# masafumiendo/benchnav

Measured on AMD Instinct MI355X. Metric: MPPI solve-steps/sec (K=1024,T=50,256x256 map), higher is better.
Workload: dtype f32

## Files before the change

benchnav_amd/csrc/mppi_capi.cpp:

```cpp
#include "mppi_handle.h"

#include <algorithm>
#include <atomic>
#include <cmath>
#include <chrono>
#include <cstdarg>
#include <cstdio>
#include <cstdlib>
#include <cstring>
#include <cerrno>
#include <sys/stat.h>
#include <fcntl.h>
#include <sys/file.h>
#include <unistd.h>
#include <map>
#include <mutex>
#include <string>
#include <vector>

namespace bn {
namespace host {

static bool wave_kernel_is_faster(const bn::SolveParams &p, size_t resident_role_wgs, int n_cus)
{
// ... 58 lines not shown
    case BN_BUF_USTAR: return B * T * 2 * 4;
    case BN_BUF_XSTAR: return B * (T + 1) * 3 * 4;
    case BN_BUF_MEAN: return B * T * 2 * 4;
    case BN_BUF_MAP: return (size_t)h->n_maps * G * G * 4;
    case BN_BUF_GOAL: return B * 2 * 4;
    case BN_BUF_USTAR_XSTAR: return (B * T * 2 + B * (T + 1) * 3) * 4;
    default: return 0;
    }
}

int ensure_scratch(bn_mppi *h, size_t bytes)
{
    if (bytes <= h->scratch_bytes) return BN_OK;
    if (h->d_scratch) BN_HIP(hipFree(h->d_scratch));
    h->d_scratch = nullptr;
    h->scratch_bytes = 0;
    BN_HIP(hipMalloc(&h->d_scratch, bytes));
    h->scratch_bytes = bytes;
    return BN_OK;
}

int flush_tail(bn_mppi *h, float *out_copy)
{
    if (h->shard_tail_inflight) {
        BN_HIP(hipStreamWaitEvent(h->stream, h->ev_shard_tail[h->shard_tail_slot], 0));
        h->shard_tail_inflight = false;
    }
    if (!h->tail_pending) return BN_OK;
    bn::SolveParams p = h->p;
    p.out_copy = out_copy;
    const int cur3 = (int)((h->solves - 1) % kSlots);
    p.part = h->d_part[cur3]; p.cost = h->d_cost[cur3]; p.state = h->d_state_copy[cur3];
    if (h->ticket_mode) {
        p.tail_merged = 1;
        p.ustar_prev = h->d_ustar2[cur3]; p.stats_prev = h->d_stats2[cur3];
    }
    p.tail_solve = h->solves - 1;
    if (h->in_episode) {
        p.env_on = 1;
        p.ep_index = h->ep_len - 1;
        p.env_z = h->ep_z ? h->ep_z + (size_t)(h->ep_len - 1) * p.B : nullptr;
    }
    p.flag_tail = h->d_flags + kSlots * (size_t)p.B * bn::kFlagStride;
    h->tails += 1;
    if (h->overlap_used) p.err_dev = reinterpret_cast<int *>(h->d_flags + ((kSlots + 1) * (size_t)p.B + 2) * bn::kFlagStride);
    if (int rc = guard_foreign_overlap(h)) return rc;
    BN_HIP(bn::launch_finish(p, h->stream));
    h->tail_pending = false;
    return BN_OK;
}

int check_instance(const bn_mppi *h, int32_t instance, bool allow_all)
{
    if (!h) return fail(BN_ERR_INVALID, "null handle");
    if (instance == -1 && allow_all) return BN_OK;
    if (instance < 0 || instance >= h->p.B)
        return fail(BN_ERR_INVALID, "instance %d out of range [0,%d)", instance, h->p.B);
    return BN_OK;
}

void journal_arm_states(bn_mppi *h)
{
    if (h->replaying) return;
    h->snap_slot = h->journal.size();
    h->arm_state_snap = h->snap_slot < h->snap_cap;
}

void journal_push(bn_mppi *h, bn_mppi::BatchRec r, bool replayable)
{
    if (h->replaying) return;
    if (!h->last_batch_overlapped && h->journal.empty()) return;
    if (!replayable || h->journal.size() >= std::min(kJournalCap, h->snap_cap) || h->snap_slot != h->journal.size()) { h->journal_lost = true; h->journal.clear(); return; }
    r.states = h->d_state_snaps + h->snap_slot * (size_t)h->p.B * 3;
    if (!h->journal_lost) h->journal.push_back(r);
}

static int recover_overlap(bn_mppi *h)
{
    for (int q = 0; q < kMaxStreams - 1; ++q)
        if (h->xstream[q]) BN_HIP(hipStreamSynchronize(h->xstream[q]));
    BN_HIP(hipStreamSynchronize(h->stream));
    BN_HIP(hipMemset(h->d_flags, 0, ((kSlots + 1) * (size_t)h->p.B + 3) * bn::kFlagStride * sizeof(unsigned long long)));
    if (h->d_ticket) BN_HIP(hipMemset(h->d_ticket, 0, (size_t)h->p.B * 65 * 4));
    for (int q = 0; q < kSlots; ++q) h->pub[q] = 0;
    h->tails = 0;
    h->prev_published = false;
    h->tail_pending = false;
#ifdef BN_EXPERIMENTS
    fprintf(stderr, "[bn] expired wait: counter %d (B=%d: [slot][b] below %d, tails above) need %d seen %d | solve %d block (%d,%d) have_prev/overlap/cur_slot %d wait_part*1000+wait_tail %d | host: solves %llu tails %llu pub %llu %llu %llu %llu\n",
            h->h_err[8], h->p.B, kSlots * h->p.B, h->h_err[9], h->h_err[10], h->h_err[11], h->h_err[12], h->h_err[13], h->h_err[14], h->h_err[15],
            (unsigned long long)h->solves, (unsigned long long)h->tails, (unsigned long long)h->pub[0], (unsigned long long)h->pub[1], (unsigned long long)h->pub[2], (unsigned long long)h->pub[kSlots - 1]);
#endif
    h->overlap_off = true;
    h->overlap_used = false;
    h->arm_snap = false;
    h->arm_state_snap = false;
    h->in_episode = false;
    *h->h_err = 0;
    std::vector<bn_mppi::BatchRec> recs;
    recs.swap(h->journal);
    const bool lost = h->journal_lost || recs.empty();
    h->journal_lost = false;
    if (lost)
        return fail(BN_ERR_HIP, "an overlapped launch gave up waiting for its predecessor's partials and the batches since the last "
                                "synchronisation point cannot be re-run: their results are invalid; this handle runs its launches on one "
                                "stream from now on");
    BN_HIP(hipMemcpy(h->d_mean, h->d_mean_snap, (size_t)h->p.B * h->p.T * 2 * 4, hipMemcpyDeviceToDevice));
    h->solves = h->journal_solves0;
    h->replaying = true;
    int rc = BN_OK;
    for (const auto &r : recs) {
        rc = r.episode ? bn_mppi_episode_async(h, r.n, r.states, BN_MEM_DEVICE, r.eps, r.noise, r.eps_ring, r.eps_stride, r.z)
                       : bn_mppi_solve_n_async(h, r.n, r.states, BN_MEM_DEVICE, r.eps, r.noise, r.eps_ring, r.eps_stride);
        if (rc != BN_OK) break;
    }
    if (rc == BN_OK) rc = flush_tail(h);
    h->replaying = false;
    if (rc != BN_OK) return rc;
    BN_HIP(hipStreamSynchronize(h->stream));
    h->recoveries += 1;
    (void)fail(BN_OK, "warning: an overlapped launch gave up waiting for its predecessor's partials; %zu batch(es) were re-run on one "
                      "stream (results are valid now; this handle no longer overlaps its launches)", recs.size());
    return BN_OK;
}

static int settle_overlap(bn_mppi *h, bool synced)
{
    if (!h->overlap_used || h->replaying) return BN_OK;
    if (__atomic_load_n(h->h_err, __ATOMIC_ACQUIRE) == 0) {
        if (synced) {
            bool idle = true;
            for (int q = 0; idle && q + 1 < h->n_streams; ++q) idle = hipStreamQuery(h->xstream[q]) == hipSuccess;
            (void)hipGetLastError();
            if (idle) { h->overlap_used = false; h->journal.clear(); h->journal_lost = false; }
        }
        return BN_OK;
    }
    return recover_overlap(h);
}

static int sync_checked(bn_mppi *h)
{
    BN_HIP(hipStreamSynchronize(h->stream));
    if (h->overlap_used)
        for (int q = 0; q + 1 < h->n_streams; ++q)
            if (h->xstream[q]) BN_HIP(hipStreamSynchronize(h->xstream[q]));
    return settle_overlap(h, true);
}

int self_check(bn_mppi *h)
{
    if (!h->self_used || h->overlap_used || h->replaying) return BN_OK;
    if (__atomic_load_n(h->h_err, __ATOMIC_ACQUIRE) == 0) return BN_OK;
    BN_HIP(hipStreamSynchronize(h->stream));
    BN_HIP(hipMemset(h->d_flags, 0, ((kSlots + 1) * (size_t)h->p.B + 3) * bn::kFlagStride * sizeof(unsigned long long)));
    for (int q = 0; q < kSlots; ++q) h->pub[q] = 0;
    h->tails = 0;
    *h->h_err = 0;
    h->self_used = false;
    h->self_off = true;
    return fail(BN_ERR_HIP, "the tail of a one-launch solve gave up waiting for the rollout workgroups of its own launch: the outputs of solve %llu "
                            "are invalid (solve again); this handle goes back to two launches per synchronous solve",
                (unsigned long long)h->solves - 1);
}

int settle_point(bn_mppi *h)
// ... 209 lines not shown
    }
    alloc(&h->d_cost_out, B * K * 4);
    alloc(&h->d_w, B * K * 4);
    alloc(&h->d_ustar, (B * T * 2 + B * (T + 1) * 3) * 4);
    if (h->d_ustar) h->d_xstar = h->d_ustar + B * T * 2;
    alloc(&h->d_stats, B * 2 * 4);
    if (rc == BN_OK && hipHostMalloc((void **)&h->h_pinned, B * 3 * 4, hipHostMallocDefault) != hipSuccess)
        rc = fail(BN_ERR_HIP, "hipHostMalloc failed");
    if (rc == BN_OK) {
        if (!(cfg->flags & BN_FLAG_PRIVATE_STREAM)) {
            h->stream = (hipStream_t)cfg->stream;
        } else if (hipStreamCreateWithFlags(&h->stream, hipStreamNonBlocking) == hipSuccess) {
            h->own_stream = true;
        } else {
            rc = fail(BN_ERR_HIP, "hipStreamCreate failed");
        }
    }
    if (rc != BN_OK) {
        bn_mppi_destroy(h);
        return rc;
    }
    p.map = h->d_map; p.state = h->d_state; p.goal = h->d_goal; p.mean = h->d_mean; p.eps = nullptr;
    p.X = h->d_X; p.U = h->d_U; p.cost = h->d_cost[0]; p.part = h->d_part[0]; p.w = h->d_w;
    p.state_copy = h->d_state_copy[0]; p.cost_out = h->d_cost_out;
    p.ustar = h->d_ustar; p.xstar = h->d_xstar; p.stats = h->d_stats; p.mean_used = h->d_mean_used;
    p.slip_on = (cfg->flags & BN_FLAG_SAMPLED_SLIP) ? 1 : 0;
    if (p.slip_on && bn::sampled_fused(p)) h->resident_wgs = bn::sampled_resident_per_cu(p) * (size_t)h->n_cus;
    h->pipelined = !h->slow_path && !(cfg->flags & BN_FLAG_NO_PIPELINE) && p.nblk <= kPipelinedMaxBlocks && !p.slip_on;
    h->wave_kernel = h->pipelined && want_wave;
    h->lat_kernel = h->pipelined && !h->wave_kernel && !(cfg->flags & BN_FLAG_ROLE_KERNEL) && bn::lat_lds_bytes(p) > 0 &&
                    ((cfg->flags & BN_FLAG_LAT_KERNEL) || ((size_t)p.B + 1) * (p.nblk + 1) <= (size_t)std::max(prop.multiProcessorCount, 1));
    if (const char *e = exp_env("BN_LAT_KERNEL")) h->lat_kernel = h->lat_kernel && e[0] != '0';
    alloc(&h->d_flags, ((kSlots + 1) * B + 3) * bn::kFlagStride * sizeof(unsigned long long));
    alloc(&h->d_mean_snap, B * T * 2 * 4);
    if (rc == BN_OK) {
        if (hipHostMalloc((void **)&h->h_err, 64, hipHostMallocMapped) != hipSuccess) rc = fail(BN_ERR_HIP, "hipHostMalloc (error word) failed");
        else if (hipHostGetDevicePointer((void **)&h->d_err, h->h_err, 0) != hipSuccess) rc = fail(BN_ERR_HIP, "hipHostGetDevicePointer failed");
        else *h->h_err = 0;
    }
    if (rc == BN_OK) {
        if (hipHostMalloc((void **)&h->h_mail, B * 2 * sizeof(unsigned long long), hipHostMallocMapped) != hipSuccess ||
            hipHostGetDevicePointer((void **)&h->d_mail, h->h_mail, 0) != hipSuccess) rc = fail(BN_ERR_HIP, "hipHostMalloc (first-action mailbox) failed");
        else std::memset(h->h_mail, 0, B * 2 * sizeof(unsigned long long));
    }
    p.mail = h->d_mail;
    if (h->lat_kernel && p.nblk <= 16 && 2 * p.T <= bn::kRolloutThreads && !exp_env("BN_NO_GRANULES"))
        for (int q = 0; q < kSlots; ++q) alloc(&h->d_gran[q], (B * (size_t)p.nblk * (2 + 2 * T) + 4 * B) * sizeof(unsigned long long));
    h->role_overlap = h->pipelined && !h->lat_kernel && !(cfg->flags & BN_FLAG_NO_OVERLAP);
    if (const char *e = exp_env("BN_ROLE_OVERLAP")) h->role_overlap = h->role_overlap && e[0] != '0';
    const bool ticket_det = !h->slow_path && !p.slip_on && !h->pipelined && !(cfg->flags & BN_FLAG_NO_PIPELINE) && p.nblk <= 1024 &&
                            bn::finish_lds_bytes(p) + 256 <= bn::rollout_lds_bytes(p);
    h->ticket_overlap = (ticket_det || (!(cfg->flags & BN_FLAG_NO_PIPELINE) && bn::sampled_fused(p))) && !(cfg->flags & BN_FLAG_NO_OVERLAP) &&
                        !exp_env("BN_NO_TICKET_OVERLAP");
    const bool may_overlap = (h->lat_kernel || h->role_overlap || h->ticket_overlap) && !(cfg->flags & BN_FLAG_NO_OVERLAP);
    if (may_overlap) {
        h->n_streams = 2;
        if (const char *e = exp_env("BN_OVERLAP_STREAMS")) h->n_streams = std::min(std::max(std::atoi(e), 2), kMaxStreams);
        for (int q = 0; q + 1 < h->n_streams; ++q) {
            if (h->d_X) alloc(&h->d_Xalt[q], B * (T + 1) * 3 * (size_t)p.Kp * 4);
            if (h->d_U) alloc(&h->d_Ualt[q], B * T * 2 * (size_t)p.Kp * 4);
        }
        h->snap_cap = std::max<size_t>(64, std::min<size_t>(4096, ((size_t)16 << 20) / ((size_t)B * 12)));
        alloc(&h->d_state_snaps, h->snap_cap * B * 3 * 4);
    }
    if (rc == BN_OK && may_overlap) {
        bool ok = hipEventCreateWithFlags(&h->ev_fork, hipEventDisableTiming) == hipSuccess;
        for (int q = 0; ok && q < h->n_streams; ++q) ok = hipEventCreateWithFlags(&h->ev_guard[q], hipEventDisableTiming) == hipSuccess;
        for (int q = 0; ok && q + 1 < h->n_streams; ++q)
            ok = hipStreamCreateWithFlags(&h->xstream[q], hipStreamNonBlocking) == hipSuccess &&
                 hipEventCreateWithFlags(&h->ev_join[q], hipEventDisableTiming) == hipSuccess;
        if (!ok) rc = fail(BN_ERR_HIP, "stream / event creation for overlapped launches failed");
    }
    if (p.slip_on) {
        alloc(&h->d_slip_std, (size_t)h->n_maps * p.G * p.G * 4);
        p.slip_std = h->d_slip_std;
        for (int q = 0; q < kSlots; ++q) {
            alloc(&h->d_ustar2[q], (size_t)p.B * p.T * 2 * 4);
            alloc(&h->d_stats2[q], (size_t)p.B * 2 * 4);
        }
        alloc(&h->d_ticket, (size_t)p.B * 65 * 4);
        alloc(&h->d_gpart, (size_t)p.B * 64 * (2 + 2 * p.T) * 4);
        p.ticket = h->d_ticket; p.gpart = h->d_gpart;
        h->ticket_mode = !h->slow_path && !(cfg->flags & BN_FLAG_NO_PIPELINE) && bn::sampled_fused(p);
    } else if (ticket_det) {
        for (int q = 0; q < kSlots; ++q) {
            alloc(&h->d_ustar2[q], (size_t)p.B * p.T * 2 * 4);
            alloc(&h->d_stats2[q], (size_t)p.B * 2 * 4);
        }
        alloc(&h->d_ticket, (size_t)p.B * 65 * 4);
        alloc(&h->d_gpart, (size_t)p.B * 64 * (2 + 2 * p.T) * 4);
        p.gpart = h->d_gpart;
        h->ticket_mode = true;
    }
    if (rc == BN_OK && !p.pow2) {
        unsigned long long *bad = h->d_flags + ((kSlots + 1) * B + 1) * bn::kFlagStride;
        const float d_max = std::max(p.x_hi - p.x0, p.y_hi - p.y0);
        unsigned long long n_bad = 1;
        if (!(std::isfinite(d_max) && d_max >= 0.0f) || bn::launch_quotient_check(p.res, p.inv_res, d_max, bad, nullptr) != hipSuccess ||
            hipMemcpy(&n_bad, bad, sizeof n_bad, hipMemcpyDeviceToHost) != hipSuccess) {
            (void)hipGetLastError();
            rc = fail(BN_ERR_HIP, "checking the cell-index quotient for resolution %g failed", (double)p.res);
        } else if (n_bad != 0) {
            rc = fail(BN_ERR_INVALID, "resolution %.9g: the correctly rounded three-instruction quotient disagrees with the division for %llu "
                                      "positions in [0, %g] (no such resolution was known: please report it); use a neighbouring value",
                      (double)p.res, n_bad, (double)d_max);
        } else {
            p.fast_div = 1;
        }
        (void)hipMemset(bad, 0, sizeof n_bad);
    }
    if (rc == BN_OK && hipDeviceSynchronize() != hipSuccess) rc = fail(BN_ERR_HIP, "hipDeviceSynchronize failed after allocation");
    if (rc == BN_OK && may_overlap) {
        int *probe = reinterpret_cast<int *>(h->d_flags + ((kSlots + 1) * B + 1) * bn::kFlagStride);
        for (int q = 0; rc == BN_OK && q + 1 < h->n_streams; ++q) {
            bool found = false;
            for (int attempt = 0; attempt < 8; ++attempt) {
                int seen = 0;
                if (hipMemset(probe, 0, 2 * sizeof(int)) != hipSuccess || bn::launch_queue_probe(probe, h->stream, h->xstream[q], h->n_cus) != hipSuccess ||
                    hipStreamSynchronize(h->stream) != hipSuccess || hipStreamSynchronize(h->xstream[q]) != hipSuccess ||
                    hipMemcpy(&seen, probe + 1, sizeof seen, hipMemcpyDeviceToHost) != hipSuccess) {
                    (void)hipGetLastError();
                    rc = fail(BN_ERR_HIP, "probing the streams of overlapped launches failed");
                    break;
                }
                if (seen) { found = true; break; }
                if (attempt == 7) break;
                hipStream_t fresh = nullptr;
                if (hipStreamCreateWithFlags(&fresh, hipStreamNonBlocking) != hipSuccess) { (void)hipGetLastError(); break; }
                h->parked.push_back(h->xstream[q]);
                h->xstream[q] = fresh;
            }
            if (exp_env("BN_DEBUG_CREATE")) std::fprintf(stderr, "[bn_mppi_create] extra stream %d: %s after %zu replacement(s)\n", q, found ? "dispatches concurrently" : "NO concurrent queue found", h->parked.size());
            if (!found && rc == BN_OK) h->overlap_off = true;
        }
        (void)hipMemset(probe, 0, 2 * sizeof(int));
    }
    if (rc == BN_OK) rc = paced_setup(h, may_overlap);
    if (rc != BN_OK) {
        bn_mppi_destroy(h);
        return rc;
    }
    {
        std::lock_guard<std::mutex> lock(g_overlap_mu);
        g_handles[h->cfg.device_id].push_back(h);
    }
    *out = h;
    return BN_OK;
}

void bn_mppi_destroy(bn_mppi_t *h)
{
    if (!h) return;
    DeviceGuard guard(h->cfg.device_id);
    hp_cancel(h);
    (void)hipStreamSynchronize(h->stream);
    {
        std::lock_guard<std::mutex> lock(g_overlap_mu);
        auto it = g_overlap_owner.find(h->cfg.device_id);
        if (it != g_overlap_owner.end() && it->second == h) g_overlap_owner.erase(it);
        g_overlap_owners.store((int)g_overlap_owner.size(), std::memory_order_relaxed);
        auto &v = g_handles[h->cfg.device_id];
        v.erase(std::remove(v.begin(), v.end(), h), v.end());
    }
    for (hipEvent_t e : h->ev) (void)hipEventDestroy(e);
    if (h->shard_comm || h->shard_prepared) shard_comm_release(h);
    env_release(h);
// ... 264 lines not shown
            p.overlap = 0;
            h->pub[cur3] += (unsigned long long)p.nblk;
            p.self_tail = 1;
            p.wait_part_self = h->pub[cur3];
            p.wait_tail_self = h->tails;
            h->tails += 1;
            p.out_copy_self = h->self_out_copy;
            if (exp_env("BN_NO_EARLY_MAIL")) p.no_early_mail = 1;
            if (h->inline_state && p.B == 1) { p.state_inline = 1; p.sv0 = h->inline_state[0]; p.sv1 = h->inline_state[1]; p.sv2 = h->inline_state[2]; }
            h->self_used = true;
            h->self_tail_launched = true;
            h->prev_published = false;
            h->hp_gran_valid = p.gran != nullptr;
            h->x_idx = 0;
        } else
        if ((h->lat_kernel || h->role_overlap) && overlap) {
            p.flag_part = h->d_flags;
            p.err = h->d_err; p.err_dev = reinterpret_cast<int *>(h->d_flags + ((kSlots + 1) * B + 2) * bn::kFlagStride);
            if (h->arm_snap) { p.mean_snap = h->d_mean_snap; h->arm_snap = false; }
            p.cur_slot = cur3; p.prev_slot = prev3;
            p.wait_part = h->pub[prev3];
            p.gran = p.lat_kernel ? h->d_gran[cur3] : nullptr;
            if (alt_buffers) {
                if (h->d_Xalt[alt_buffers - 1]) p.X = h->d_Xalt[alt_buffers - 1];
                if (h->d_Ualt[alt_buffers - 1] && p.U) p.U = h->d_Ualt[alt_buffers - 1];
            }
            p.overlap = (h->prev_published && p.have_prev) ? 1 : 0;
            p.gran_prev = (p.overlap && p.lat_kernel) ? h->d_gran[prev3] : nullptr;
            if (on_stream) st = on_stream;
            if (p.overlap) h->overlap_used = true;
            h->pub[cur3] += (unsigned long long)p.nblk;
            h->prev_published = true;
            if (self_tail && p.lat_kernel && !h->in_episode) {
                p.self_tail = 1;
                p.wait_part_self = h->pub[cur3];
                p.wait_tail_self = h->tails;
                h->tails += 1;
            }
        } else {
            h->prev_published = false;
        }
        p.aux_prio = (!p.wave_kernel && (size_t)p.B * (p.nblk + 1) > h->resident_wgs) ? 1 : 0;
        if (!p.wave_kernel && !p.store_u) p.U = nullptr;
        if (p.self_tail) BN_HIP(bn::launch_rollout_lat_self(p, mode, st));
        else BN_HIP(bn::launch_rollout(p, mode, st));
        if (st != h->stream && lone_self) {
            BN_HIP(hipEventRecord(h->hp_ev[h->hp_redo_q], st));
            BN_HIP(hipStreamWaitEvent(h->stream, h->hp_ev[h->hp_redo_q], 0));
        }
        if (prof_grouped) h->prof_in_group = (h->prof_in_group + 1) % kProfGroup;
        h->solves += 1;
        h->x_idx = 0;
        h->tail_pending = !p.self_tail;
        if (p.self_tail) h->prev_published = false;
        if (lone_self) h->last_batch_overlapped = false;
        return BN_OK;
    }
    if (!(h->ticket_overlap && overlap && !shard_rollout)) h->prev_published = false;
    p.have_prev = 0;
    p.mean_from_part = 0;
    p.tail_solve = p.solve;
    if (p.slip_on && !h->slip_std_set) return fail(BN_ERR_STATE, "bn_mppi_set_slip_std must precede solve in sampled-slip mode");
    if (h->ticket_mode && !shard_rollout) {
        p.have_prev = h->tail_pending ? 1 : 0;
        p.tail_merged = 1;
        p.tail_solve = p.solve - 1;
        p.ustar_cur = h->d_ustar2[cur3]; p.stats_cur = h->d_stats2[cur3];
        p.ustar_prev = h->d_ustar2[prev3]; p.stats_prev = h->d_stats2[prev3];
        p.ticket = h->d_ticket;
        hipStream_t st = h->stream;
        p.flag_tail = h->d_flags + kSlots * B * bn::kFlagStride;
        if (p.have_prev) { p.wait_tail = h->tails; h->tails += 1; }
        if (h->ticket_overlap && overlap) {
            p.flag_part = h->d_flags;
            p.err = h->d_err; p.err_dev = reinterpret_cast<int *>(h->d_flags + ((kSlots + 1) * B + 2) * bn::kFlagStride);
            if (h->arm_snap) { p.mean_snap = h->d_mean_snap; h->arm_snap = false; }
            p.cur_slot = cur3; p.prev_slot = prev3;
            p.wait_part = h->pub[prev3];
            if (alt_buffers) {
                if (h->d_Xalt[alt_buffers - 1]) p.X = h->d_Xalt[alt_buffers - 1];
                if (h->d_Ualt[alt_buffers - 1] && p.U) p.U = h->d_Ualt[alt_buffers - 1];
            }
            p.overlap = (h->prev_published && p.have_prev) ? 1 : 0;
            if (on_stream) st = on_stream;
            if (p.overlap) h->overlap_used = true;
            h->pub[cur3] += 1;
            h->prev_published = true;
        }
        if (p.slip_on) BN_HIP(bn::launch_rollout_sampled(p, mode, st));
        else BN_HIP(bn::launch_rollout(p, mode, st));
        if (prof_grouped) h->prof_in_group = (h->prof_in_group + 1) % kProfGroup;
        h->solves += 1;
        h->tail_pending = true;
        return BN_OK;
    }
    if (shard_rollout && h->shard_inplace) p.part = h->d_gathered + (size_t)h->shard_rank * p.nblk * (2 + 2 * T);
    if (p.slip_on) {
        BN_HIP(bn::launch_rollout_sampled(p, mode, h->stream));
    } else {
        if (h->slow_path) p.wave_kernel = 1;
        else if (!p.store_u) p.U = nullptr;
        BN_HIP(bn::launch_rollout(p, mode, h->stream));
    }
    if (prof) BN_HIP(hipEventRecord(ev[1], h->stream));
    if (shard_rollout) {
        if (prof) BN_HIP(hipEventRecord(ev[2], h->stream));
        h->solves += 1;
        h->tail_pending = false;
        h->shard_pending = true;
        return BN_OK;
    }
    p.state = p.state_copy;
    BN_HIP(bn::launch_finish(p, h->stream));
    if (prof) BN_HIP(hipEventRecord(ev[2], h->stream));
    h->solves += 1;
    h->tail_pending = false;
    return BN_OK;
}

}
}

extern "C" {

int bn_mppi_solve_async(bn_mppi_t *h, const float *states, bn_mem_kind states_where, const float *eps,
                        bn_noise_kind noise)
{
    if (h && !h->replaying && !h->journal.empty()) {
        h->last_batch_overlapped = false;
        journal_arm_states(h);
        journal_push(h, bn_mppi::BatchRec{1, states, eps, noise, 1, 0, false, nullptr}, states_where == BN_MEM_DEVICE && noise != BN_NOISE_HOST_KT2);
    }
    return solve_impl(h, states, states_where, eps, noise, false);
}

int bn_mppi_solve_n_async(bn_mppi_t *h, int32_t n, const float *states, bn_mem_kind states_where, const float *eps,
                          bn_noise_kind noise, int32_t eps_ring, int64_t eps_stride)
{
    if (n < 0) return fail(BN_ERR_INVALID, "n must be >= 0");
    if (eps && (eps_ring < 1 || eps_stride < 0)) return fail(BN_ERR_INVALID, "eps_ring must be >= 1 and eps_stride >= 0");
    if (!h) return fail(BN_ERR_INVALID, "null handle");
    const bool overlap = (h->lat_kernel || h->role_overlap || h->ticket_overlap) && h->n_streams > 1 && (h->d_Xalt[0] || h->p.lean) && n >= 3 && states_where == BN_MEM_DEVICE &&
                         noise != BN_NOISE_HOST_KT2 && !(h->cfg.flags & (BN_FLAG_PROFILE | BN_FLAG_NO_OVERLAP)) && !h->shard_pending && !h->overlap_off;
    int mode = overlap ? h->tune.chosen : 1;
    if (overlap && h->tune.explore && n >= 128 && !h->in_episode && !h->replaying) {
        const int32_t ring = eps ? eps_ring : 1;
        const int32_t prefix = ((192 + ring - 1) / ring) * ring;
        if (n > prefix + 2) {
            if (int rc = bn_mppi_solve_n_async(h, prefix, states, states_where, eps, noise, eps_ring, eps_stride)) return rc;
            h->tune.explore = 0;
            return bn_mppi_solve_n_async(h, n - prefix, states, states_where, eps, noise, eps_ring, eps_stride);
        }
        mode = 1 - h->tune.chosen;
    }
    if (mode != h->run_mode) h->ov_sample.valid = false;
    h->run_mode = mode;
    bool mine = overlap && mode == 0;
    if (mine) {
        BN_BIND(h);
        std::lock_guard<std::mutex> lock(g_overlap_mu);
        bn_mppi *&owner = g_overlap_owner[h->cfg.device_id];
        if (owner && owner != h) {
            bool busy = hipStreamQuery(owner->stream) != hipSuccess;
            for (int q = 0; !busy && q + 1 < owner->n_streams; ++q) busy = hipStreamQuery(owner->xstream[q]) != hipSuccess;
            (void)hipGetLastError();
            if (busy) mine = false;
// ... 162 lines not shown
```

benchnav_amd/csrc/rollout_sampled.hip:

```cpp
#include "mppi_device.h"

namespace bn {

namespace {

constexpr int kSampledWaves = 8;
constexpr int kSampledThreads = 64 * kSampledWaves;

__host__ __device__ inline size_t sampled_lds_floats(int T, int WN)
{
    const size_t TP = (size_t)((T + 2) & ~1);
    return 4 * 64 * (size_t)(T + 1) + 2 * (size_t)WN * WN + 2 * 64 * TP + 2 * (size_t)T * kUPad + 4 * (size_t)T + 128;
}

template <int EPS, int GEO, bool STORE_U>
__global__ __launch_bounds__(kSampledThreads) void rollout_sampled_kernel(const SolveParams p)
{
    extern __shared__ __attribute__((aligned(16))) float smem[];
    const int T = p.T, K = p.K, WN2 = p.WN * p.WN;
    const int TP = (T + 2) & ~1;
    float4 *XL = reinterpret_cast<float4 *>(smem);
    float2 *win2 = reinterpret_cast<float2 *>(smem + 4 * 64 * (T + 1));
    float *Zt = reinterpret_cast<float *>(win2 + WN2), *Zc = Zt + 64 * TP;
    float *Ul = Zc + 64 * TP, *ml = Ul + 2 * T * kUPad, *mv = ml + 2 * T, *el = mv + 2 * T, *ad = el + 64;
    const WgId wg = decode_wg(p);
    if (wg.idle) return;
    const int tid = threadIdx.x, lane = tid & 63, b = wg.b;
    if (wg.aux) {
        if (p.overlap) finish_body<GEO, true, kSampledThreads, false, true>(p, b, nullptr, p.cost_prev, p.state_prev, smem);
        else finish_body<GEO, true, kSampledThreads>(p, b, nullptr, p.cost_prev, p.state_prev, smem);
        return;
    }
    const int wid = __builtin_amdgcn_readfirstlane(tid >> 6);
    const int k = wg.blk * 64 + lane;
    const bool active = k < K;
    const int kk = active ? k : K - 1;
    const float *__restrict__ mu = p.map + (size_t)b * p.map_stride;
    const float *__restrict__ sg = p.slip_std + (size_t)b * p.map_stride;
    const float sx = p.state[b * 3 + 0], sy = p.state[b * 3 + 1], sth = p.state[b * 3 + 2];
    const float gx = p.goal[b * 2 + 0], gy = p.goal[b * 2 + 1];
    const Win w = window_origin<GEO>(p, sx, sy);
    const size_t Kp = (size_t)p.Kp;
    float *Xb = p.X + (size_t)b * (T + 1) * 3 * Kp + k;
    float *Ub = STORE_U ? p.U + (size_t)b * T * 2 * Kp + k : nullptr;

    BN_STAMP(0);
    for (int e = tid; e < WN2; e += kSampledThreads) {
        const int r = e / p.WN, c = e - r * p.WN;
        const size_t g = (size_t)min(w.wy0 + r, p.G - 1) * p.G + min(w.wx0 + c, p.G - 1);
        win2[e] = make_float2(mu[g], sg[g]);
    }
    const bool ovs = p.overlap != 0;
    const bool tpub = p.flag_part != nullptr;
    if (!ovs)
    for (int j = tid; j < 2 * T; j += kSampledThreads) {
        const float m = p.mean[(size_t)b * 2 * T + j];
        ml[j] = m;
        mv[j] = m * ((j & 1) ? p.iv1 : p.iv0);
    }
    if (wg.blk == 0 && tid < 3) { if (tpub) store_agent(p.state_copy + b * 3 + tid, p.state[b * 3 + tid]); else p.state_copy[b * 3 + tid] = p.state[b * 3 + tid]; }
    if (p.state_snap && wg.blk == 0 && tid < 3) p.state_snap[b * 3 + tid] = p.state[b * 3 + tid];
    __syncthreads();

    {
        const int nE = (T + 1) >> 1, nS = TP >> 1;
        for (int q = nE + wid; q < nE + nS; q += kSampledWaves) {
            {
                const int r0 = 2 * (q - nE), r1 = r0 + 1;
                float z[4];
                if (p.zt) {
                    z[0] = r0 < T ? p.zt[((size_t)b * T + r0) * K + kk] : 0.0f;
                    z[1] = r1 < T ? p.zt[((size_t)b * T + r1) * K + kk] : 0.0f;
                    z[2] = r0 <= T ? p.zc[((size_t)b * (T + 1) + r0) * K + kk] : 0.0f;
                    z[3] = r1 <= T ? p.zc[((size_t)b * (T + 1) + r1) * K + kk] : 0.0f;
                } else {
                    philox_slip_block(p.seed, p.solve, (uint32_t)b, (uint32_t)(kk + p.k0), (uint32_t)(q - nE), z);
                }
                Zt[r0 * 64 + lane] = z[0]; Zt[r1 * 64 + lane] = z[1];
                Zc[r0 * 64 + lane] = z[2]; Zc[r1 * 64 + lane] = z[3];
            }
        }
        if (ovs) {
            if (tid == 0) wait_counter<16>(flag_ctr(p.flag_part, p.prev_slot * p.B + b), p.wait_part, p);
            __syncthreads();
            for (int j = tid; j < 2 * T; j += kSampledThreads) {
                const float m = load_agent(p.mean + (size_t)b * 2 * T + j);
                ml[j] = m;
                mv[j] = m * ((j & 1) ? p.iv1 : p.iv0);
            }
            __syncthreads();
        }
        if (p.mean_snap && wg.blk == 0 && wid == 0) snapshot_mean(p, b, ml, lane);
        for (int q = wid; q < nE; q += kSampledWaves) produce_pair<EPS, STORE_U>(p, p.eps, b, kk, 2 * q, p.solve, ml, Ul, Ub, Kp, lane);
    }
    __syncthreads();
    BN_STAMP(1);

    if (wid == 0) {
        SlipChain c;
        c.x = sx; c.y = sy; c.th = sth;
        sincos_spec(c.th, c.sn, c.cs);
        c.e = slip_cell_safe<GEO, true>(p, w, sx, sy);
        float xn, yn, tn;
        slip_chain_step<GEO, true>(p, win2, w, c, Ul[lane], Ul[kUPad + lane], Zt[lane], xn, yn, tn);
        XL[lane] = make_float4(xn, yn, tn, __int_as_float(c.e));
        int t = 1;
        for (; t + 4 <= T; t += 4) {
            float uq[4][3];
#pragma unroll
            for (int i = 0; i < 4; ++i) {
                uq[i][0] = Ul[(2 * (t + i)) * kUPad + lane]; uq[i][1] = Ul[(2 * (t + i) + 1) * kUPad + lane];
                uq[i][2] = Zt[(t + i) * 64 + lane];
            }
#pragma unroll
            for (int i = 0; i < 4; ++i) {
                slip_chain_step<GEO, false>(p, win2, w, c, uq[i][0], uq[i][1], uq[i][2], xn, yn, tn);
                __builtin_amdgcn_sched_barrier(0);
                XL[(t + i) * 64 + lane] = make_float4(xn, yn, tn, __int_as_float(c.e));
            }
        }
        for (; t < T; ++t) {
            slip_chain_step<GEO, false>(p, win2, w, c, Ul[(2 * t) * kUPad + lane], Ul[(2 * t + 1) * kUPad + lane], Zt[t * 64 + lane],
                                        xn, yn, tn);
            XL[t * 64 + lane] = make_float4(xn, yn, tn, __int_as_float(c.e));
        }
        XL[T * 64 + lane] = make_float4(c.x, c.y, c.th, __int_as_float(c.e));
    } else if (wid == 1) {
        double Ad = 0.0;
        for (int t = 0; t < T; ++t)
            Ad += (double)(p.lambda_ * (mv[2 * t] * Ul[(2 * t) * kUPad + lane] + mv[2 * t + 1] * Ul[(2 * t + 1) * kUPad + lane]));
        ad[lane] = (float)Ad;
    }
    __syncthreads();
    BN_STAMP(2);

    for (int t = wid; t <= T; t += kSampledWaves) {
        const float4 o = XL[t * 64 + lane];
        float *Xt = Xb + (size_t)(3 * t) * Kp;
        Xt[0] = o.x; Xt[Kp] = o.y; Xt[2 * Kp] = o.z;
        const float2 ms = win2[__float_as_int(o.w)];
        const float tc = trav_from_slip(ms.x, ms.y, Zc[t * 64 + lane]);
        const float dx = o.x - gx, dy = o.y - gy;
        Zc[t * 64 + lane] = sqrt_cr_normal(dx * dx + dy * dy) + (tc <= p.thr ? 1.0e4f : 0.0f);
    }
    __syncthreads();
    BN_STAMP(3);

    if (wid == 0) {
        double Sd = 0.0;
#pragma unroll 16
        for (int t = 0; t < T; ++t) Sd += (double)Zc[t * 64 + lane];
        const float cost = ((float)Sd + Zc[T * 64 + lane]) + ad[lane];
        if (active) { if (tpub) store_agent(p.cost + (size_t)b * K + k, cost); else p.cost[(size_t)b * K + k] = cost; }
        const float zz = active ? (-cost) / p.lambda_ : -INFINITY;
        const float zmax = wave_max(zz);
        const float e = active ? expf(zz - zmax) : 0.0f;
        const float esum = wave_sum(e);
        el[lane] = e;
        if (lane == 0) {
            float *part = p.part + ((size_t)b * p.nblk + wg.blk) * (2 + 2 * T);
            store_agent(part, zmax); store_agent(part + 1, esum);
        }
    }
    __syncthreads();
    column_sums<kSampledThreads, true>(Ul, el, T, tid, p.part + ((size_t)b * p.nblk + wg.blk) * (2 + 2 * T));
    BN_STAMP(5);
    if (p.ustar_cur) ticket_merge<kSampledThreads>(p, b, wg.blk, smem);
}

template <int EPS, int GEO, bool STORE_U>
__global__ __launch_bounds__(64) void rollout_sampled_global_kernel(const SolveParams p)
{
    extern __shared__ __attribute__((aligned(16))) float smem[];
    const int T = p.T, K = p.K;
    float *ml = smem, *mv = ml + 2 * T, *Ul = mv + 2 * T, *el = Ul + 2 * T * kUPad;
    const WgId wg = decode_wg(p);
    if (wg.idle) return;
    const int lane = threadIdx.x, b = wg.b;
    const int k = wg.blk * 64 + lane;
    const bool active = k < K;
    const int kk = active ? k : K - 1;
    const float *__restrict__ mu = p.map + (size_t)b * p.map_stride;
    const float *__restrict__ sg = p.slip_std + (size_t)b * p.map_stride;
    const float sx = p.state[b * 3 + 0], sy = p.state[b * 3 + 1], sth = p.state[b * 3 + 2];
    const float gx = p.goal[b * 2 + 0], gy = p.goal[b * 2 + 1];
    const Win w{0, 0, 0.f, 0.f, 0.f, 0.f};
    for (int j = lane; j < 2 * T; j += 64) {
        const float m = p.mean[(size_t)b * 2 * T + j];
        ml[j] = m;
        mv[j] = m * ((j & 1) ? p.iv1 : p.iv0);
    }
    if (wg.blk == 0 && lane < 3) p.state_copy[b * 3 + lane] = p.state[b * 3 + lane];
    if (p.state_snap && wg.blk == 0 && lane < 3) p.state_snap[b * 3 + lane] = p.state[b * 3 + lane];
    __syncthreads();
    const size_t Kp = (size_t)p.Kp;
    float *Xb = p.X + (size_t)b * (T + 1) * 3 * Kp + k;
    float *Ub = STORE_U ? p.U + (size_t)b * T * 2 * Kp + k : nullptr;
    for (int t = 0; t < T; t += 2) produce_pair<EPS, STORE_U>(p, p.eps, b, kk, t, p.solve, ml, Ul, Ub, Kp, lane);
    __syncthreads();
    float x = sx, y = sy, th = sth;
    float sn, cs;
    sincos_spec(th, sn, cs);
    float zq[4] = {0.f, 0.f, 0.f, 0.f};
    double Sd = 0.0, Ad = 0.0;
    for (int t = 0; t < T; ++t) {
        if (p.zt) {
            zq[t & 1] = p.zt[((size_t)b * T + t) * K + kk];
            zq[2 + (t & 1)] = p.zc[((size_t)b * (T + 1) + t) * K + kk];
        } else if ((t & 1) == 0) {
            philox_slip_block(p.seed, p.solve, (uint32_t)b, (uint32_t)(kk + p.k0), (uint32_t)(t >> 1), zq);
        }
        const float u0 = Ul[(2 * t) * kUPad + lane], u1 = Ul[(2 * t + 1) * kUPad + lane];
        const int e = slip_cell_safe<GEO, false>(p, w, x, y);
        const float trav = trav_from_slip(mu[e], sg[e], zq[t & 1]);
        float xn, yn, tn;
        if (p.ref_order) {
            sincos_spec(th, sn, cs);
            const float tv = trav * u0;
            xn = x + (tv * cs) * p.dt; yn = y + (tv * sn) * p.dt;
            tn = th + (trav * u1) * p.dt;
            th = wrap_angle(tn);
        } else {
            const float g = u0 * p.dt, dth = trav * (u1 * p.dt);
            xn = __builtin_fmaf(trav, g * cs, x); yn = __builtin_fmaf(trav, g * sn, y);
            tn = theta_step(th, dth, t == 0);
            rotate_spec(cs, sn, dth);
        }
        float *Xt = Xb + (size_t)(3 * t) * Kp;
        Xt[0] = xn; Xt[Kp] = yn; Xt[2 * Kp] = tn;
        x = clampf(xn, p.x0, p.x_hi); y = clampf(yn, p.y0, p.y_hi);
        const int ec = slip_cell_safe<GEO, false>(p, w, xn, yn);
        const float tc = trav_from_slip(mu[ec], sg[ec], zq[2 + (t & 1)]);
        const float dx = xn - gx, dy = yn - gy;
        Sd += (double)(sqrt_cr_normal(dx * dx + dy * dy) + (tc <= p.thr ? 1.0e4f : 0.0f));
        Ad += (double)(p.lambda_ * (mv[2 * t] * u0 + mv[2 * t + 1] * u1));
    }
    {
        float *Xt = Xb + (size_t)(3 * T) * Kp;
        Xt[0] = x; Xt[Kp] = y; Xt[2 * Kp] = th;
    }
    if (p.zt) zq[2 + (T & 1)] = p.zc[((size_t)b * (T + 1) + T) * K + kk];
    else if ((T & 1) == 0) philox_slip_block(p.seed, p.solve, (uint32_t)b, (uint32_t)(kk + p.k0), (uint32_t)(T >> 1), zq);
    const int eT = slip_cell_safe<GEO, false>(p, w, x, y);
    const float tT = trav_from_slip(mu[eT], sg[eT], zq[2 + (T & 1)]);
    const float dxT = x - gx, dyT = y - gy;
    const float term = sqrt_cr_normal(dxT * dxT + dyT * dyT) + (tT <= p.thr ? 1.0e4f : 0.0f);
    const float cost = ((float)Sd + term) + (float)Ad;
    if (active) p.cost[(size_t)b * K + k] = cost;
    const float zz = active ? (-cost) / p.lambda_ : -INFINITY;
    const float zmax = wave_max(zz);
// ... 105 lines not shown
```

Measured before the change: 107,700.

## Pipeline sampled rollout waves via LDS progress slots and granule-based mean handoff

Inside the sampled rollout kernel, the chain wave now posts per-step progress to an LDS counter. Cost accumulation and trajectory stores run on other waves as soon as slots are ready, which removes two block-wide barrier phases. Noise drawing is moved ahead of the wait for the previous solve's mean, and the mean arrives through tagged per-element granules polled by 128 threads instead of a single counter wait. A custom merge publishes these granules. The change adds spin-wait complexity, extra device buffers and reset logic, and a risk of ordering bugs between waves and across overlapped solves.

After: 96820. 0.899x the previous value.

```diff
diff --git a/benchnav_amd/csrc/mppi_capi.cpp b/benchnav_amd/csrc/mppi_capi.cpp
--- a/benchnav_amd/csrc/mppi_capi.cpp
+++ b/benchnav_amd/csrc/mppi_capi.cpp
@@ -164,6 +164,9 @@
     BN_HIP(hipStreamSynchronize(h->stream));
     BN_HIP(hipMemset(h->d_flags, 0, ((kSlots + 1) * (size_t)h->p.B + 3) * bn::kFlagStride * sizeof(unsigned long long)));
     if (h->d_ticket) BN_HIP(hipMemset(h->d_ticket, 0, (size_t)h->p.B * 65 * 4));
+    if (h->ticket_mode && h->p.slip_on)
+        for (int q = 0; q < kSlots; ++q)
+            if (h->d_gran[q]) BN_HIP(hipMemset(h->d_gran[q], 0, (size_t)h->p.B * 2 * h->p.T * sizeof(unsigned long long)));
     for (int q = 0; q < kSlots; ++q) h->pub[q] = 0;
     h->tails = 0;
     h->prev_published = false;
@@ -539,6 +542,8 @@
         alloc(&h->d_gpart, (size_t)p.B * 64 * (2 + 2 * p.T) * 4);
         p.ticket = h->d_ticket; p.gpart = h->d_gpart;
         h->ticket_mode = !h->slow_path && !(cfg->flags & BN_FLAG_NO_PIPELINE) && bn::sampled_fused(p);
+        if (h->ticket_mode)
+            for (int q = 0; q < kSlots; ++q) alloc(&h->d_gran[q], (size_t)p.B * 2 * p.T * sizeof(unsigned long long));
     } else if (ticket_det) {
         for (int q = 0; q < kSlots; ++q) {
             alloc(&h->d_ustar2[q], (size_t)p.B * p.T * 2 * 4);
@@ -969,6 +974,10 @@
                 if (h->d_Ualt[alt_buffers - 1] && p.U) p.U = h->d_Ualt[alt_buffers - 1];
             }
             p.overlap = (h->prev_published && p.have_prev) ? 1 : 0;
+            if (p.slip_on) {
+                p.gran = h->d_gran[cur3];
+                p.gran_prev = p.overlap ? h->d_gran[prev3] : nullptr;
+            }
             if (on_stream) st = on_stream;
             if (p.overlap) h->overlap_used = true;
             h->pub[cur3] += 1;
diff --git a/benchnav_amd/csrc/rollout_sampled.hip b/benchnav_amd/csrc/rollout_sampled.hip
--- a/benchnav_amd/csrc/rollout_sampled.hip
+++ b/benchnav_amd/csrc/rollout_sampled.hip
@@ -10,7 +10,171 @@
 __host__ __device__ inline size_t sampled_lds_floats(int T, int WN)
 {
     const size_t TP = (size_t)((T + 2) & ~1);
-    return 4 * 64 * (size_t)(T + 1) + 2 * (size_t)WN * WN + 2 * 64 * TP + 2 * (size_t)T * kUPad + 4 * (size_t)T + 128;
+    return 4 * 64 * (size_t)(T + 1) + 2 * (size_t)WN * WN + 2 * 64 * TP + 2 * (size_t)T * kUPad + 4 * (size_t)T + 128 + 4;
+}
+
+template <int EPS>
+__device__ __forceinline__ void draw_pair(const SolveParams &p, int b, int kk, int t, float *Ul, int lane)
+{
+    float e[4];
+    noise_pair<EPS>(p, b, kk, t, e);
+#pragma unroll
+    for (int s = 0; s < 2; ++s)
+        if (t + s < p.T) {
+            Ul[(2 * (t + s)) * kUPad + lane] = e[2 * s];
+            Ul[(2 * (t + s) + 1) * kUPad + lane] = e[2 * s + 1];
+        }
+}
+
+template <bool STORE_U>
+__device__ __forceinline__ void shape_pair(const SolveParams &p, int t, const float *ml, float *Ul, float *Ub, size_t Kp, int lane)
+{
+#pragma unroll
+    for (int s = 0; s < 2; ++s) {
+        const int tt = t + s;
+        if (tt < p.T) {
+            const float u0 = clampf(ml[2 * tt] + p.sigma0 * Ul[(2 * tt) * kUPad + lane], p.umin0, p.umax0);
+            const float u1 = clampf(ml[2 * tt + 1] + p.sigma1 * Ul[(2 * tt + 1) * kUPad + lane], p.umin1, p.umax1);
+            Ul[(2 * tt) * kUPad + lane] = u0;
+            Ul[(2 * tt + 1) * kUPad + lane] = u1;
+            if (STORE_U) { float *Ut = Ub + (size_t)(2 * tt) * Kp; Ut[0] = u0; Ut[Kp] = u1; }
+        }
+    }
+}
+
+constexpr int kMeanPollThreads = 128;
+__device__ __forceinline__ void mean_from_granules(const SolveParams &p, int b, int tid, float *ml, float *mv)
+{
+    const int n = 2 * p.T;
+    const unsigned long long *g = p.gran_prev + (size_t)b * n;
+    const uint32_t tag = (uint32_t)p.solve;
+    for (int j0 = 0; j0 < n; j0 += kMeanPollThreads) {
+        const int j = j0 + tid;
+        bool ok = j >= n;
+        float v = 0.0f;
+        for (int it = 0;; ++it) {
+            if (!ok) { bool k = true; v = load_granule(g + j, tag, k); ok = k; }
+            if (__all(ok)) break;
+            if (it >= (1 << 23) / 16 + 1024) { if ((tid & 63) == 0) raise_wait_expired(p, nullptr, 903); break; }
+            __builtin_amdgcn_s_sleep(16);
+        }
+        if (j < n) { ml[j] = v; mv[j] = v * ((j & 1) ? p.iv1 : p.iv0); }
+    }
+}
+
+typedef __attribute__((address_space(3))) volatile int lds_vint;
+__device__ __forceinline__ void post_slots(int *prog, int n)
+{
+    asm volatile("" ::: "memory");
+    *(lds_vint *)prog = n;
+}
+template <int SLEEP = 1>
+__device__ __forceinline__ int wait_slots(int *prog, int need)
+{
+    lds_vint *p3 = (lds_vint *)prog;
+    int n = *p3;
+    while (n < need) { __builtin_amdgcn_s_sleep(SLEEP); n = *p3; }
+    asm volatile("" ::: "memory");
+    return n;
+}
+
+template <int GEO, bool STEP_POST>
+__device__ __forceinline__ void chain_chunk(const SolveParams &p, const float2 *win2, const Win &w, SlipChain &c, const float *Ul,
+                                            const float *Zt, float4 *XL, int *prog, int t, int lane)
+{
+    float uq[4][3], xn, yn, tn;
+#pragma unroll
+    for (int i = 0; i < 4; ++i) {
+        uq[i][0] = Ul[(2 * (t + i)) * kUPad + lane]; uq[i][1] = Ul[(2 * (t + i) + 1) * kUPad + lane];
+        uq[i][2] = Zt[(t + i) * 64 + lane];
+    }
+#pragma unroll
+    for (int i = 0; i < 4; ++i) {
+        slip_chain_step<GEO, false>(p, win2, w, c, uq[i][0], uq[i][1], uq[i][2], xn, yn, tn);
+        __builtin_amdgcn_sched_barrier(0);
+        XL[(t + i) * 64 + lane] = make_float4(xn, yn, tn, __int_as_float(c.e));
+        if (STEP_POST) post_slots(prog, t + i + 1);
+    }
+    if (!STEP_POST) post_slots(prog, t + 4);
+}
+
+__device__ __forceinline__ float slot_cost(const SolveParams &p, const float4 *XL, const float2 *win2, const float *Zc, int t, int lane,
+                                           float gx, float gy)
+{
+    const float4 o = XL[t * 64 + lane];
+    const float2 ms = win2[__float_as_int(o.w)];
+    const float tc = trav_from_slip(ms.x, ms.y, Zc[t * 64 + lane]);
+    const float dx = o.x - gx, dy = o.y - gy;
+    return sqrt_cr_normal(dx * dx + dy * dy) + (tc <= p.thr ? 1.0e4f : 0.0f);
+}
+
+constexpr int kFlatRows = 8 * kGroupRows;
+
+template <int NT>
+__device__ __forceinline__ void sampled_merge(const SolveParams &p, int b, int blk, float *scratch)
+{
+    const int T = p.T, tid = threadIdx.x, PS = 2 + 2 * p.T;
+    const bool flat = p.nblk > 64 && p.nblk <= kFlatRows;
+    float *us = scratch, *sc = us + 2 * T, *red = sc + p.nblk;
+    int *flag = reinterpret_cast<int *>(red + 32 + (flat ? ((p.nblk + kGroupRows - 1) / kGroupRows) * PS : 0));
+    int *ticket = p.ticket + (size_t)b * kTicketStride;
+    const float *part = p.part + (size_t)b * p.nblk * PS;
+    const float *rows = part;
+    int nrows = p.nblk;
+    if (p.nblk > kFlatRows) {
+        const int g = blk / kGroupRows, ng = (p.nblk + kGroupRows - 1) / kGroupRows;
+        const int in_group = min(kGroupRows, p.nblk - g * kGroupRows);
+        asm volatile("s_waitcnt vmcnt(0)" ::: "memory");
+        __syncthreads();
+        if (tid == 0) *flag = (atomicAdd(ticket + 1 + g, 1) == in_group - 1) ? 1 : 0;
+        __syncthreads();
+        if (!*flag) return;
+        if (tid == 0) __hip_atomic_store(ticket + 1 + g, 0, __ATOMIC_RELAXED, __HIP_MEMORY_SCOPE_AGENT);
+        float *grow = p.gpart + ((size_t)b * 64 + g) * PS;
+        merge_group<true, true>(part, g * kGroupRows, in_group, T, tid & 63, tid >> 6, NT / 64, grow);
+        rows = p.gpart + (size_t)b * 64 * PS;
+        nrows = ng;
+    }
+    asm volatile("s_waitcnt vmcnt(0)" ::: "memory");
+    __syncthreads();
+    if (tid == 0) *flag = (atomicAdd(ticket, 1) == nrows - 1) ? 1 : 0;
+    __syncthreads();
+    if (!*flag) return;
+    BN_STAMP_ANY(6);
+    if (tid == 0) __hip_atomic_store(ticket, 0, __ATOMIC_RELAXED, __HIP_MEMORY_SCOPE_AGENT);
+    float m, S;
+    if (flat) merge_partials<NT, true, true>(part, p.nblk, T, us, sc, red, tid, m, S, false, MergeLoads{});
+    else merge_partials<NT, true, false>(rows, nrows, T, us, sc, red, tid, m, S, false, MergeLoads{});
+    const bool pubm = p.flag_part != nullptr;
+    if (pubm && p.gran) {
+        asm volatile("s_waitcnt vmcnt(0)" ::: "memory");
+        __syncthreads();
+        for (int j = tid; j < 2 * T; j += NT) store_granule(p.gran + (size_t)b * 2 * T + j, us[j], (uint32_t)p.solve + 1u);
+    }
+    if (p.overlap && p.gran_prev) {
+        if (tid == 0) wait_counter(flag_ctr(p.flag_part, p.prev_slot * p.B + b), p.wait_part, p);
+        __syncthreads();
+    }
+    const bool spoiled = pubm && batch_spoiled(p);
+    for (int j = tid; j < 2 * T; j += NT) {
+        const size_t at = (size_t)b * 2 * T + j;
+        if (pubm) {
+            store_agent(p.ustar_cur + at, us[j]);
+            if (spoiled) continue;
+            if (p.mean_used) store_agent(p.mean_used + at, load_agent(p.mean + at));
+            store_agent(p.mean + at, us[j]);
+        } else {
+            p.ustar_cur[at] = us[j];
+            if (p.mean_used) p.mean_used[at] = p.mean[at];
+            p.mean[at] = us[j];
+        }
+    }
+    if (tid == 0) {
+        if (pubm) { store_agent(p.stats_cur + b * 2 + 0, m); store_agent(p.stats_cur + b * 2 + 1, S); }
+        else { p.stats_cur[b * 2 + 0] = m; p.stats_cur[b * 2 + 1] = S; }
+    }
+    if (pubm) publish_counter(flag_ctr(p.flag_part, p.cur_slot * p.B + b), tid);
+    BN_STAMP_ANY(7);
 }
 
 template <int EPS, int GEO, bool STORE_U>
@@ -23,6 +187,7 @@
     float2 *win2 = reinterpret_cast<float2 *>(smem + 4 * 64 * (T + 1));
     float *Zt = reinterpret_cast<float *>(win2 + WN2), *Zc = Zt + 64 * TP;
     float *Ul = Zc + 64 * TP, *ml = Ul + 2 * T * kUPad, *mv = ml + 2 * T, *el = mv + 2 * T, *ad = el + 64;
+    int *prog = reinterpret_cast<int *>(ad + 64);
     const WgId wg = decode_wg(p);
     if (wg.idle) return;
     const int tid = threadIdx.x, lane = tid & 63, b = wg.b;
@@ -58,6 +223,7 @@
         ml[j] = m;
         mv[j] = m * ((j & 1) ? p.iv1 : p.iv0);
     }
+    if (tid < 2) prog[tid] = 0;
     if (wg.blk == 0 && tid < 3) { if (tpub) store_agent(p.state_copy + b * 3 + tid, p.state[b * 3 + tid]); else p.state_copy[b * 3 + tid] = p.state[b * 3 + tid]; }
     if (p.state_snap && wg.blk == 0 && tid < 3) p.state_snap[b * 3 + tid] = p.state[b * 3 + tid];
     __syncthreads();
@@ -65,22 +231,27 @@
     {
         const int nE = (T + 1) >> 1, nS = TP >> 1;
         for (int q = nE + wid; q < nE + nS; q += kSampledWaves) {
-            {
-                const int r0 = 2 * (q - nE), r1 = r0 + 1;
-                float z[4];
-                if (p.zt) {
-                    z[0] = r0 < T ? p.zt[((size_t)b * T + r0) * K + kk] : 0.0f;
-                    z[1] = r1 < T ? p.zt[((size_t)b * T + r1) * K + kk] : 0.0f;
-                    z[2] = r0 <= T ? p.zc[((size_t)b * (T + 1) + r0) * K + kk] : 0.0f;
-                    z[3] = r1 <= T ? p.zc[((size_t)b * (T + 1) + r1) * K + kk] : 0.0f;
-                } else {
-                    philox_slip_block(p.seed, p.solve, (uint32_t)b, (uint32_t)(kk + p.k0), (uint32_t)(q - nE), z);
-                }
-                Zt[r0 * 64 + lane] = z[0]; Zt[r1 * 64 + lane] = z[1];
-                Zc[r0 * 64 + lane] = z[2]; Zc[r1 * 64 + lane] = z[3];
+            const int r0 = 2 * (q - nE), r1 = r0 + 1;
+            float z[4];
+            if (p.zt) {
+                z[0] = r0 < T ? p.zt[((size_t)b * T + r0) * K + kk] : 0.0f;
+                z[1] = r1 < T ? p.zt[((size_t)b * T + r1) * K + kk] : 0.0f;
+                z[2] = r0 <= T ? p.zc[((size_t)b * (T + 1) + r0) * K + kk] : 0.0f;
+                z[3] = r1 <= T ? p.zc[((size_t)b * (T + 1) + r1) * K + kk] : 0.0f;
+            } else {
+                philox_slip_block(p.seed, p.solve, (uint32_t)b, (uint32_t)(kk + p.k0), (uint32_t)(q - nE), z);
             }
-        }
-        if (ovs) {
+            Zt[r0 * 64 + lane] = z[0]; Zt[r1 * 64 + lane] = z[1];
+            Zc[r0 * 64 + lane] = z[2]; Zc[r1 * 64 + lane] = z[3];
+        }
+        for (int q = wid; q < nE; q += kSampledWaves) {
+            if (ovs) draw_pair<EPS>(p, b, kk, 2 * q, Ul, lane);
+            else produce_pair<EPS, STORE_U>(p, p.eps, b, kk, 2 * q, p.solve, ml, Ul, Ub, Kp, lane);
+        }
+        if (ovs && p.gran_prev) {
+            if (tid < kMeanPollThreads) mean_from_granules(p, b, tid, ml, mv);
+            __syncthreads();
+        } else if (ovs) {
             if (tid == 0) wait_counter<16>(flag_ctr(p.flag_part, p.prev_slot * p.B + b), p.wait_part, p);
             __syncthreads();
             for (int j = tid; j < 2 * T; j += kSampledThreads) {
@@ -91,7 +262,8 @@
             __syncthreads();
         }
         if (p.mean_snap && wg.blk == 0 && wid == 0) snapshot_mean(p, b, ml, lane);
-        for (int q = wid; q < nE; q += kSampledWaves) produce_pair<EPS, STORE_U>(p, p.eps, b, kk, 2 * q, p.solve, ml, Ul, Ub, Kp, lane);
+        if (ovs)
+            for (int q = wid; q < nE; q += kSampledWaves) shape_pair<STORE_U>(p, 2 * q, ml, Ul, Ub, Kp, lane);
     }
     __syncthreads();
     BN_STAMP(1);
@@ -104,53 +276,37 @@
         float xn, yn, tn;
         slip_chain_step<GEO, true>(p, win2, w, c, Ul[lane], Ul[kUPad + lane], Zt[lane], xn, yn, tn);
         XL[lane] = make_float4(xn, yn, tn, __int_as_float(c.e));
+        post_slots(prog, 1);
         int t = 1;
-        for (; t + 4 <= T; t += 4) {
-            float uq[4][3];
-#pragma unroll
-            for (int i = 0; i < 4; ++i) {
-                uq[i][0] = Ul[(2 * (t + i)) * kUPad + lane]; uq[i][1] = Ul[(2 * (t + i) + 1) * kUPad + lane];
-                uq[i][2] = Zt[(t + i) * 64 + lane];
-            }
-#pragma unroll
-            for (int i = 0; i < 4; ++i) {
-                slip_chain_step<GEO, false>(p, win2, w, c, uq[i][0], uq[i][1], uq[i][2], xn, yn, tn);
-                __builtin_amdgcn_sched_barrier(0);
-                XL[(t + i) * 64 + lane] = make_float4(xn, yn, tn, __int_as_float(c.e));
-            }
-        }
+        for (; t + 8 <= T; t += 4) chain_chunk<GEO, false>(p, win2, w, c, Ul, Zt, XL, prog, t, lane);
+        if (t + 4 <= T) { chain_chunk<GEO, true>(p, win2, w, c, Ul, Zt, XL, prog, t, lane); t += 4; }
         for (; t < T; ++t) {
             slip_chain_step<GEO, false>(p, win2, w, c, Ul[(2 * t) * kUPad + lane], Ul[(2 * t + 1) * kUPad + lane], Zt[t * 64 + lane],
                                         xn, yn, tn);
             XL[t * 64 + lane] = make_float4(xn, yn, tn, __int_as_float(c.e));
+            post_slots(prog, t + 1);
         }
         XL[T * 64 + lane] = make_float4(c.x, c.y, c.th, __int_as_float(c.e));
+        post_slots(prog, T + 1);
+        BN_STAMP(2);
     } else if (wid == 1) {
-        double Ad = 0.0;
-        for (int t = 0; t < T; ++t)
-            Ad += (double)(p.lambda_ * (mv[2 * t] * Ul[(2 * t) * kUPad + lane] + mv[2 * t + 1] * Ul[(2 * t + 1) * kUPad + lane]));
-        ad[lane] = (float)Ad;
-    }
-    __syncthreads();
-    BN_STAMP(2);
-
-    for (int t = wid; t <= T; t += kSampledWaves) {
-        const float4 o = XL[t * 64 + lane];
-        float *Xt = Xb + (size_t)(3 * t) * Kp;
-        Xt[0] = o.x; Xt[Kp] = o.y; Xt[2 * Kp] = o.z;
-        const float2 ms = win2[__float_as_int(o.w)];
-        const float tc = trav_from_slip(ms.x, ms.y, Zc[t * 64 + lane]);
-        const float dx = o.x - gx, dy = o.y - gy;
-        Zc[t * 64 + lane] = sqrt_cr_normal(dx * dx + dy * dy) + (tc <= p.thr ? 1.0e4f : 0.0f);
-    }
-    __syncthreads();
-    BN_STAMP(3);
-
-    if (wid == 0) {
         double Sd = 0.0;
-#pragma unroll 16
-        for (int t = 0; t < T; ++t) Sd += (double)Zc[t * 64 + lane];
-        const float cost = ((float)Sd + Zc[T * 64 + lane]) + ad[lane];
+        int t = 0;
+        while (t < T) {
+            const int n = min(wait_slots(prog, t + 1), T);
+            for (; t + 4 <= n; t += 4) {
+                float sc4[4];
+#pragma unroll
+                for (int i = 0; i < 4; ++i) sc4[i] = slot_cost(p, XL, win2, Zc, t + i, lane, gx, gy);
+#pragma unroll
+                for (int i = 0; i < 4; ++i) Sd += (double)sc4[i];
+            }
+            for (; t < n; ++t) Sd += (double)slot_cost(p, XL, win2, Zc, t, lane, gx, gy);
+        }
+        wait_slots(prog, T + 1);
+        const float term = slot_cost(p, XL, win2, Zc, T, lane, gx, gy);
+        wait_slots(prog + 1, 1);
+        const float cost = ((float)Sd + term) + ad[lane];
         if (active) { if (tpub) store_agent(p.cost + (size_t)b * K + k, cost); else p.cost[(size_t)b * K + k] = cost; }
         const float zz = active ? (-cost) / p.lambda_ : -INFINITY;
         const float zmax = wave_max(zz);
@@ -161,11 +317,28 @@
             float *part = p.part + ((size_t)b * p.nblk + wg.blk) * (2 + 2 * T);
             store_agent(part, zmax); store_agent(part + 1, esum);
         }
-    }
-    __syncthreads();
+    } else {
+        if (wid == 2) {
+            double Ad = 0.0;
+            for (int t = 0; t < T; ++t)
+                Ad += (double)(p.lambda_ * (mv[2 * t] * Ul[(2 * t) * kUPad + lane] + mv[2 * t + 1] * Ul[(2 * t + 1) * kUPad + lane]));
+            ad[lane] = (float)Ad;
+            post_slots(prog + 1, 1);
+        }
+        if (wid != 4)
+        for (int t = wid - (wid > 4 ? 3 : 2); t <= T; t += kSampledWaves - 3) {
+            wait_slots<4>(prog, t + 1);
+            const float4 o = XL[t * 64 + lane];
+            float *Xt = Xb + (size_t)(3 * t) * Kp;
+            Xt[0] = o.x; Xt[Kp] = o.y; Xt[2 * Kp] = o.z;
+        }
+    }
+    __syncthreads();
+    BN_STAMP(3);
+
     column_sums<kSampledThreads, true>(Ul, el, T, tid, p.part + ((size_t)b * p.nblk + wg.blk) * (2 + 2 * T));
     BN_STAMP(5);
-    if (p.ustar_cur) ticket_merge<kSampledThreads>(p, b, wg.blk, smem);
+    if (p.ustar_cur) sampled_merge<kSampledThreads>(p, b, wg.blk, smem);
 }
 
 template <int EPS, int GEO, bool STORE_U>
```
